# lucidrains/glom-pytorch

Hardware: NVIDIA H100
Metric: column-iterations/sec (BxNxLxiters) at dim=512 L=6 224/14 (higher is better)
Workload: dtype bf16

## Files before the change

glom_pytorch_b200/_native.py:

```python
import ctypes
import os

_PKG = os.path.dirname(os.path.abspath(__file__))
LIB_PATH = os.environ.get("GLOM_B200_LIB") or os.path.join(_PKG, "libglom_b200.so")

ABI_VERSION = 1
PRECISION = {"fp32": 0, "bf16": 1}
PROFILE_KINDS = ("attention", "gemm1_gelu", "gemm2_combine", "prologue", "tokenize")


class Cfg(ctypes.Structure):
    _fields_ = [("struct_size", ctypes.c_uint32), ("dim", ctypes.c_int32), ("levels", ctypes.c_int32),
                ("n", ctypes.c_int32), ("attend_self", ctypes.c_int32), ("mask_side", ctypes.c_int32),
                ("mask_d2_max", ctypes.c_int32), ("precision", ctypes.c_int32)]


class WeightsRef(ctypes.Structure):
    _fields_ = [("struct_size", ctypes.c_uint32)] + [
        (k, ctypes.c_void_p) for k in ("bu_w1", "bu_b1", "bu_w2", "bu_b2", "td_w1", "td_b1", "td_w2", "td_b2")]


class Grads(ctypes.Structure):
    _fields_ = [("struct_size", ctypes.c_uint32)] + [
        (k, ctypes.c_void_p) for k in ("d_tokens", "d_pos", "d_state0", "d_init", "d_bu_w1", "d_bu_b1", "d_bu_w2",
                                       "d_bu_b2", "d_td_w1", "d_td_b1", "d_td_w2", "d_td_b2")]


_vp, _sz, _i32, _f32 = ctypes.c_void_p, ctypes.c_size_t, ctypes.c_int, ctypes.c_float
_CFG, _W, _G = ctypes.POINTER(Cfg), ctypes.POINTER(WeightsRef), ctypes.POINTER(Grads)
_SZP, _I32P = ctypes.POINTER(_sz), ctypes.POINTER(_i32)
_SETTLE = [_CFG, _vp, _vp, _vp, _vp, _vp, _vp, _i32, _i32, _f32, _vp, _vp, _sz, _vp]

SIGNATURES = {
    "glom_b200_abi_version": (_i32, []),
    "glom_b200_last_error": (ctypes.c_char_p, []),
    "glom_b200_packed_weight_bytes": (_i32, [_CFG, _SZP]),
    "glom_b200_pack_weights": (_i32, [_CFG, _W, _vp, _sz, _vp]),
    "glom_b200_workspace_bytes": (_i32, [_CFG, _i32, _i32, _i32, _SZP]),
    "glom_b200_forward": (_i32, [_CFG, _vp, _vp, _vp, _vp, _vp, _vp, _i32, _i32, _i32, _vp, _sz, _vp]),
    "glom_b200_forward_resume": (_i32, [_CFG, _vp, _vp, _vp, _vp, _vp, _i32, _i32, _i32, _vp, _sz, _vp, _i32, _I32P]),
    "glom_b200_settle_workspace_bytes": (_i32, [_CFG, _i32, _i32, _SZP]),
    "glom_b200_settle": (_i32, _SETTLE),
    "glom_b200_settle_all_workspace_bytes": (_i32, [_CFG, _i32, _i32, _SZP]),
    "glom_b200_settle_all": (_i32, _SETTLE),
    "glom_b200_settle_workspace_offset": (_i32, [_CFG, _i32, _i32, _i32, _i32, _SZP, _SZP]),
    "glom_b200_settle_queue_workspace_bytes": (_i32, [_CFG, _i32, _i32, _SZP]),
    "glom_b200_settle_queue_begin": (_i32, [_CFG, _vp, _vp, _vp, _vp, _vp, _vp, _i32, _i32, _i32, _f32, _vp, _sz, _vp]),
    "glom_b200_settle_queue_run": (_i32, [_CFG, _vp, _vp, _vp, _vp, _vp, _vp, _vp, _i32, _i32, _i32, _f32, _vp, _sz, _vp,
                                          _i32, _i32, _vp]),
    "glom_b200_settle_video_workspace_bytes": (_i32, [_CFG, _i32, _i32, _SZP]),
    "glom_b200_settle_video_begin": (_i32, [_CFG, _vp, _vp, _vp, _vp, _vp, _vp, _i32, _i32, _i32, _i32, _f32, _vp, _sz,
                                            _vp]),
    "glom_b200_settle_video_run": (_i32, [_CFG, _vp, _vp, _vp, _vp, _vp, _vp, _vp, _i32, _i32, _i32, _i32, _f32, _vp, _sz,
                                          _vp, _i32, _i32, _vp]),
    "glom_b200_forward_steps_workspace_bytes": (_i32, [_CFG, _i32, _i32, _i32, _SZP]),
    "glom_b200_forward_steps": (_i32, [_CFG, _vp, _vp, _vp, _vp, _vp, _vp, _i32, _vp, _i32, _i32, _vp, _sz, _vp]),
    "glom_b200_tokenize_workspace_bytes": (_i32, [_i32, _i32, _i32, _i32, _i32, _i32, _SZP]),
    "glom_b200_tokenize": (_i32, [_vp, _vp, _vp, _vp, _i32, _i32, _i32, _i32, _i32, _i32, _vp, _sz, _vp]),
    "glom_b200_last_launch_count": (_i32, []),
    "glom_b200_workspace_offset": (_i32, [_CFG, _i32, _i32, _i32, _i32, _SZP, _SZP]),
    "glom_b200_backward_workspace_bytes": (_i32, [_CFG, _i32, _SZP]),
# ... 50 lines not shown
    if rc != 0:
        raise GlomB200Error(f"glom_b200 error {rc}: {load().glom_b200_last_error().decode()}")


def make_cfg(dim, levels, n, attend_self, mask_side, mask_d2_max, precision):
    return Cfg(ctypes.sizeof(Cfg), dim, levels, n, int(bool(attend_self)), mask_side, mask_d2_max,
               PRECISION[precision])


def _bytes(symbol, *args):
    out = ctypes.c_size_t()
    check(getattr(load(), symbol)(*args, ctypes.byref(out)))
    return out.value


def packed_weight_bytes(cfg):
    return _bytes("glom_b200_packed_weight_bytes", ctypes.byref(cfg))


def workspace_bytes(cfg, batch, iters, return_all):
    return _bytes("glom_b200_workspace_bytes", ctypes.byref(cfg), batch, iters, int(return_all))


def workspace_offset(cfg, batch, iters, return_all, which):
    off, nb = ctypes.c_size_t(), ctypes.c_size_t()
    check(load().glom_b200_workspace_offset(ctypes.byref(cfg), batch, iters, int(return_all), which,
                                            ctypes.byref(off), ctypes.byref(nb)))
    return off.value, nb.value


def settle_workspace_offset(cfg, batch, max_iters, return_all, which):
    off, nb = ctypes.c_size_t(), ctypes.c_size_t()
    check(load().glom_b200_settle_workspace_offset(ctypes.byref(cfg), batch, max_iters, int(return_all), which,
                                                   ctypes.byref(off), ctypes.byref(nb)))
    return off.value, nb.value


def pack_weights(cfg, ptrs, packed_ptr, packed_bytes, stream):
    w = WeightsRef(ctypes.sizeof(WeightsRef), *ptrs)
    check(load().glom_b200_pack_weights(ctypes.byref(cfg), ctypes.byref(w), packed_ptr, packed_bytes, stream))


def forward(cfg, packed_ptr, tokens_ptr, pos_ptr, state_in_ptr, init_ptr, out_ptr, batch, iters,
            return_all, ws_ptr, ws_bytes, stream):
    check(load().glom_b200_forward(ctypes.byref(cfg), packed_ptr, tokens_ptr, pos_ptr, state_in_ptr, init_ptr,
                                   out_ptr, batch, iters, int(return_all), ws_ptr, ws_bytes, stream))
# ... 176 lines not shown
```

glom_pytorch_b200/csrc/engine.h:

```cpp
#pragma once
#include <cuda.h>
#include <cuda_runtime.h>
#include <cuda_bf16.h>
#include <stdarg.h>
#include <stddef.h>
#include <stdint.h>
#include <stdio.h>
#include <atomic>
#include <mutex>
#include <vector>

#include "../../include/glom_b200.h"

namespace glom {

enum ProfKind { PROF_ATTN = 0, PROF_GEMM1 = 1, PROF_GEMM2 = 2, PROF_PREP = 3, PROF_TOKENIZE = 4, PROF_KINDS = 5 };
struct Profiler {
  bool enabled = false;
  std::vector<cudaEvent_t> ev;
  size_t used = 0;
  struct Span { int kind; size_t a, b; };
  std::vector<Span> spans;
  size_t mark(cudaStream_t st) {
    if (used == ev.size()) { cudaEvent_t e; cudaEventCreate(&e); ev.push_back(e); }
// ... 22 lines not shown

struct PackedLayout {
  size_t w1_off, w2_off, b1_off, b2_off, total;
};
PackedLayout packed_layout(int d, int L, int precision);

struct WorkspaceLayout {
  size_t s32_off;
  size_t s32_bytes;
  size_t sb_off[2];
  size_t sp_off[2];
  size_t xb_off;
  size_t h_off;
  size_t h_bytes;
  size_t c_off;
  size_t c_bytes;
  size_t nsq_off[2];
  size_t nsq_bytes;
  size_t attn_acc_off;
  size_t attn_acc_bytes;
  size_t total;
};
WorkspaceLayout workspace_layout(const Geometry& g, int precision, int iters, int return_all);

struct SettleLayout {
  WorkspaceLayout fwd;
  size_t dsq_off;
  size_t flags_off;
  size_t frozen_off;
  size_t block_frozen_off;
  size_t done_off;
  size_t level_q_off;
  size_t flags_bytes;
  size_t total;
};
SettleLayout settle_layout(const Geometry& g, int max_iters, int return_all = 0);

struct QueueLayout {
  SettleLayout settle;
  size_t slab_off[2];
  size_t queue_off;
  size_t slot_img_off;
  size_t age_off;
  size_t pending_off;
  size_t gather_off;
  size_t fresh_off;
// ... 6 lines not shown
QueueLayout queue_layout(const Geometry& g, int max_iters);

struct QueueSlots {
  int *slot_img, *age, *pending, *gather_img, *fresh, *block_fresh, *head, *unfinished;
  int images, frames, max_iters;
};

struct Bf16Buffers {
  const float* s32_in;  float* s32_out;
  int s32_in_bcast;
  const __nv_bfloat16* sb_in;  __nv_bfloat16* sb_out;
  const __nv_bfloat16* sp_in;  __nv_bfloat16* sp_out;
  const __nv_bfloat16* xb;
  __nv_bfloat16* h;  __nv_bfloat16* c;
  float* attn_acc;
  const float* nsq_in;  float* nsq_out;
  const float* pos;
  const __nv_bfloat16* w1;  const __nv_bfloat16* w2;  const float* b1;  const float* b2;
  const int* frozen;
  const int* block_frozen;
  float* dsq_out;
  const int* block_fresh;
  int ii_reduce;
};

static inline int rep_h_blocks(int n) {
  int a = n, b = 128;
  while (b) { const int r = a % b; a = b; b = r; }
  return n / a;
}
static inline int rep_row_blocks(int n) { return (rep_h_blocks(n) * 128 + 255) / 256; }

typedef CUresult (*EncodeTiledFn)(CUtensorMap*, CUtensorMapDataType, cuuint32_t, void*, const cuuint64_t*,
                                  const cuuint64_t*, const cuuint32_t*, const cuuint32_t*, CUtensorMapInterleave,
                                  CUtensorMapSwizzle, CUtensorMapL2promotion, CUtensorMapFloatOOBfill);

struct Launch {
  EncodeTiledFn enc; int num_sms; cudaStream_t st; Profiler* prof;
  int launches;
  char err[400];
  int launched(cudaError_t e, const char* what = nullptr) { ++launches; return check(e, what); }
  int launched(const char* what = nullptr) { return launched(cudaGetLastError(), what); }
  int check(cudaError_t e, const char* what = nullptr) {
    if (e == cudaSuccess) return 0;
    return what ? fail(GLOM_B200_ERR_CUDA, "%s: %s", what, cudaGetErrorString(e)) : fail(GLOM_B200_ERR_CUDA, "%s", cudaGetErrorString(e));
  }
// ... 166 lines not shown
```

glom_pytorch_b200/csrc/gemm_sched.cuh:

```cuda
#pragma once
#include "tc_common.cuh"

namespace glom {

struct GemmParams {
  int rows, d, L, n, G;
  int num_m, num_n, num_tiles;
  int m128;
  int z0;
  int n_half;
  const float* bias;
  const float* s32_in;
  int s_bcast;
  const __nv_bfloat16* c_in;
  const float* pos;
  float* s32_out;
  __nv_bfloat16* sb_out;
  __nv_bfloat16* sp_out;
  float* nsq_out;
  int nparts;
  float* tok_out;
  int tok_kb;
  const int* frozen;
  const int* block_frozen;
  float* dsq_out;
  const int* block_fresh;
  int num_m_rep, num_full_tiles;
  unsigned long long full_mask, rep_mask;
  int remap_l, h_period;
};

struct TileInfo {
  int z;
  int m_blk, n_blk;
  int num_kb;
};

__host__ __device__ __forceinline__ int nth_set_bit(unsigned long long m, int k) {
  int z = 0;
  for (;; ++z)
    if ((m >> z) & 1ull) { if (k == 0) return z; --k; }
}

template <int MODE, bool REDUCED = false>
__host__ __device__ __forceinline__ TileInfo decode_tile(const GemmParams& p, int tile) {
  TileInfo t;
  if (REDUCED && p.num_m_rep > 0) {
    const bool full = tile < p.num_full_tiles;
    const int nm = full ? p.num_m : p.num_m_rep;
    const int r = full ? tile / p.num_n : (tile - p.num_full_tiles) / p.num_n;
    t.n_blk = tile % p.num_n;
    t.m_blk = r % nm;
    t.z = nth_set_bit(full ? p.full_mask : p.rep_mask, r / nm);
  } else {
    t.n_blk = tile % p.num_n;
    const int r = tile / p.num_n;
    t.m_blk = r % p.num_m;
    t.z = p.z0 + r / p.num_m;
  }
  if (MODE == 0) t.num_kb = p.d / BK;
  else if (MODE == 1) t.num_kb = ((t.z == p.L - 1) ? 4 * p.d : 8 * p.d) / BK;
  else t.num_kb = p.tok_kb;
  return t;
}

template <int MODE>
__host__ __device__ __forceinline__ int sched_tile(const GemmParams& p, int c, int C, int it) {
  if (MODE != 1) { const int t = c + it * C; return t < p.num_tiles ? t : -1; }
  const int S = p.n_half;
  const int B = p.num_tiles - S;
  const int heavy = B % C;
  const int nb = (B - c + C - 1) / C;
  const int nbig = nb > 0 ? nb : 0;
  if (it < nbig) return c + it * C;
  int k = it - nbig;
  const int light = C - heavy;
  const int first = (2 * light < S) ? 2 * light : S;
  if (c >= heavy) {
    if (k < 2) { const int j = k * light + (c - heavy); if (j < first) return B + j; }
    k -= 2;
    if (k < 0) return -1;
  }
  const int j = first + k * C + c;
  return j < S ? B + j : -1;
}

__host__ __device__ __forceinline__ bool ii_k1_full(int z, int t) { return (z & 1) ? z <= 2 * t - 3 : z <= 2 * t; }
__host__ __device__ __forceinline__ bool ii_k2_full(int l, int t) { return l <= t; }
__host__ __device__ __forceinline__ int ii_k3_full_levels(int t) { return t; }

template <typename Full>
__host__ __forceinline__ void set_reduced(GemmParams& p, int z_end, int num_m_rep, Full full) {
  p.num_m_rep = num_m_rep;
  p.full_mask = p.rep_mask = 0;
  for (int z = p.z0; z < z_end; ++z) (full(z) ? p.full_mask : p.rep_mask) |= 1ull << z;
  p.num_full_tiles = __builtin_popcountll(p.full_mask) * p.num_m * p.num_n;
  p.num_tiles = p.num_full_tiles + __builtin_popcountll(p.rep_mask) * num_m_rep * p.num_n;
}

__host__ __device__ __forceinline__ void attn_item(int it, int full_items, int per_img, int ntiles, int l_full, int& b, int& l) {
  if (it >= full_items) { b = 0; l = l_full + (it - full_items) / ntiles; }
  else { b = it / per_img; l = (it % per_img) / ntiles; }
}

}
```

glom_pytorch_b200/csrc/glom_api.cu:

```cuda
#include "../../include/glom_b200.h"
#include "../../include/glom_b200_tree.h"
#include "engine.h"

#include <mutex>
#include <stdarg.h>
#include <stdio.h>
#include <string.h>

namespace glom {

static thread_local char g_err[512] = "";
static thread_local Profiler g_prof;
static thread_local Launch g_launch{};

static int fail(int code, const char* fmt, ...) {
  va_list ap;
  va_start(ap, fmt);
  vsnprintf(g_err, sizeof(g_err), fmt, ap);
  va_end(ap);
  return code;
}

static bool misaligned(const void* p, size_t a) { return reinterpret_cast<uintptr_t>(p) % a != 0; }

// ... 17 lines not shown
  w.s32_off = off;
  w.s32_bytes = (return_all || iters == 0) ? 0 : state_elems * 4;
  off = align_up(off + w.s32_bytes, 1024);
  if (precision == GLOM_B200_BF16) {
    for (int i = 0; i < 2; ++i) { w.sb_off[i] = off; off = align_up(off + state_elems * 2, 1024); }
    for (int i = 0; i < 2; ++i) { w.sp_off[i] = off; off = align_up(off + (size_t)g.rows * (g.L - 1) * g.d * 2, 1024); }
    w.xb_off = off; off = align_up(off + (size_t)g.rows * g.d * 2, 1024);
    w.h_bytes = (size_t)((g.rows + 127) / 128 * 128) * g.G * 4 * g.d * 2;
    w.c_bytes = state_elems * 2;
    w.nsq_bytes = (size_t)g.rows * g.L * g.nparts * 4;
  } else {
    w.h_bytes = (size_t)g.rows * g.G * 4 * g.d * 4;
    w.c_bytes = state_elems * 4;
    w.nsq_bytes = 0;
  }
  w.h_off = off; off = align_up(off + w.h_bytes, 1024);
  w.c_off = off; off = align_up(off + w.c_bytes, 1024);
  for (int i = 0; i < 2; ++i) { w.nsq_off[i] = off; off = align_up(off + w.nsq_bytes, 1024); }
  w.attn_acc_off = off;
  w.attn_acc_bytes = (precision == GLOM_B200_BF16 && g.n > 576) ? (state_elems + (size_t)g.rows * g.L * 2) * 4 : 0;
  off = align_up(off + w.attn_acc_bytes, 1024);
  w.total = off > 0 ? off : 1024;
  return w;
}

SettleLayout settle_layout(const Geometry& g, int max_iters, int return_all) {
  SettleLayout s{};
  s.fwd = workspace_layout(g, GLOM_B200_BF16, max_iters, return_all);
  size_t off = s.fwd.total;
  s.dsq_off = off; off = align_up(off + s.fwd.nsq_bytes, 1024);
  s.flags_off = off;
  s.frozen_off = off; off = align_up(off + (size_t)g.B * 4, 16);
  s.block_frozen_off = off; off = align_up(off + (size_t)(g.rows + 255) / 256 * 4, 16);
  s.done_off = off; off = align_up(off + 4, 16);
  s.level_q_off = off; off += (size_t)g.B * g.L * 4;
  s.flags_bytes = off - s.flags_off;
  s.total = align_up(off, 1024);
  return s;
}

QueueLayout queue_layout(const Geometry& g, int max_iters) {
  QueueLayout q{};
  q.settle = settle_layout(g, max_iters, 0);
  size_t off = q.settle.total;
  q.slab_off[0] = q.settle.fwd.s32_off;
  q.slab_off[1] = off; off = align_up(off + q.settle.fwd.s32_bytes, 1024);
// ... 108 lines not shown
  return 0;
}

GLOM_B200_API int glom_b200_pack_weights(const glom_b200_cfg* cfg, const glom_b200_weights_ref* w, void* packed, size_t packed_bytes,
                           void* stream) {
  if (int r = check_cfg(cfg)) return r;
  if (!w || w->struct_size != sizeof(glom_b200_weights_ref)) return fail(GLOM_B200_ERR_INVALID, "weights struct missing or wrong size");
  if (!w->bu_w1 || !w->bu_b1 || !w->bu_w2 || !w->bu_b2 || !w->td_w1 || !w->td_b1 || !w->td_w2 || !w->td_b2)
    return fail(GLOM_B200_ERR_INVALID, "a weight pointer is NULL");
  const PackedLayout pl = packed_layout(cfg->dim, cfg->levels, cfg->precision);
  if (!packed || packed_bytes < pl.total) return fail(GLOM_B200_ERR_WORKSPACE, "packed buffer: need %zu bytes, got %zu", pl.total, packed_bytes);
  if (misaligned(packed, 1024)) return fail(GLOM_B200_ERR_INVALID, "packed buffer must be 1024-byte aligned");
  Launch& ln = begin_launch(0, stream);
  if (int r = launch_pack(cfg->dim, cfg->levels, cfg->precision, w->bu_w1, w->bu_b1, w->bu_w2, w->bu_b2, w->td_w1, w->td_b1,
                          w->td_w2, w->td_b2, packed, ln))
    return fail(r, "pack_weights launch: %s", ln.err);
  return 0;
}

GLOM_B200_API int glom_b200_workspace_bytes(const glom_b200_cfg* cfg, int batch, int iters, int return_all, size_t* out_bytes) {
  if (int r = check_cfg(cfg)) return r;
  if (batch < 1 || iters < 0 || !out_bytes) return fail(GLOM_B200_ERR_INVALID, "bad batch/iters/out_bytes");
  *out_bytes = workspace_layout(make_geometry(cfg, batch), cfg->precision, iters, return_all).total;
  return 0;
}

GLOM_B200_API int glom_b200_workspace_offset(const glom_b200_cfg* cfg, int batch, int iters, int return_all, int which,
                               size_t* out_offset, size_t* out_bytes) {
  if (int r = check_cfg(cfg)) return r;
  if (batch < 1 || iters < 0 || !out_offset || !out_bytes) return fail(GLOM_B200_ERR_INVALID, "bad arguments");
  const WorkspaceLayout w = workspace_layout(make_geometry(cfg, batch), cfg->precision, iters, return_all);
  switch (which) {
    case 0: *out_offset = w.h_off; *out_bytes = w.h_bytes; return 0;
    case 1: *out_offset = w.c_off; *out_bytes = w.c_bytes; return 0;
    case 2: *out_offset = w.nsq_off[0]; *out_bytes = w.nsq_bytes; return 0;
    default: return fail(GLOM_B200_ERR_INVALID, "unknown workspace buffer id %d", which);
  }
}


static int check_tensors(const char* pre, bool has_packed, const void* packed_weights, const float* tokens, const float* pos,
                         const float* state_in, const float* init_levels, const float* state_out, const void* workspace) {
  if ((has_packed && !packed_weights) || !tokens || !pos || !state_out)
    return fail(GLOM_B200_ERR_INVALID, "%sa required pointer is NULL", pre);
  if (!state_in && !init_levels) return fail(GLOM_B200_ERR_INVALID, "%sneed state_in or init_levels", pre);
  if (state_in == state_out) return fail(GLOM_B200_ERR_INVALID, "%sstate_out must not alias state_in", pre);
// ... 96 lines not shown
    Bf16Buffers& b = sbuf.step;
    const bool resume = a.resume_parity >= 0;
    const int p0 = resume ? a.resume_parity : 0;
    const bool s0_direct = resume || (!return_all && iters >= 1);
    int prep;
    if (resume) {
      prep = launch_prep(g, nullptr, nullptr, a.pos, a.tokens, nullptr, nullptr, nullptr, sbuf.xb, nullptr, ln);
      if (prep == 0 && return_all)
        prep = ln.launched(cudaMemcpyAsync(state_out, state_in, slab * sizeof(float), cudaMemcpyDeviceToDevice, ln.st));
    } else {
      prep = launch_prep(g, state_in, init_levels, a.pos, a.tokens, s0_direct ? nullptr : loc(0), sbuf.sb[0], sbuf.sp[0], sbuf.xb,
                         sbuf.nsq[0], ln);
    }
    if (prep) return fail(prep, "prep launch: %s", ln.err);
    const SettleFlags fl = freeze ? bind_settle_flags(sl, a.workspace) : SettleFlags{};
    b.frozen = fl.frozen; b.block_frozen = fl.block_frozen;
    b.dsq_out = settle ? fl.dsq : nullptr;
    if (settle) {
      if (int r = ln.check(cudaMemsetAsync(ws + sl.flags_off, 0, sl.flags_bytes, ln.st)))
        return fail(r, "settle flags memset: %s", ln.err);
    }
    const bool ii = !state_in && !resume && !freeze && iters >= g.L + 1 && g.L <= 32 &&
                    rep_row_blocks(g.n) < (g.rows + 255) / 256 && (size_t)g.n * g.L * g.d < (1u << 31);
    for (int t = 0; t < iters; ++t) {
      if (steps) {
        if (int r = launch_steps_schedule(g, t, iters, steps, fl.frozen, fl.block_frozen, ln))
          return fail(r, "step schedule launch before step %d: %s", t, ln.err);
      }
      b.s32_in = (s0_direct && t == 0) ? (state_in ? state_in : init_levels) : loc(t); b.s32_out = loc(t + 1);
      b.s32_in_bcast = (s0_direct && t == 0 && !state_in) ? 1 : 0;
      set_parity(sbuf, (t + p0) & 1);
      b.ii_reduce = ii && t < g.L;
      if (int r = step_bf16(g, b, t, ln)) return fail(r, "step %d: %s", t, ln.err);
      if (settle) {
        if (int r = launch_settle_converge(g, t + 1, settle->tol, fl.dsq, b.nsq_out, fl.frozen, fl.block_frozen, fl.done,
                                           fl.level_q, settle->steps, ln))
          return fail(r, "settle convergence launch after step %d: %s", t, ln.err);
      }
    }
    const int32_t* image_steps = settle ? settle->steps : steps;
    if (ii && return_all) {
      if (int r = launch_level_fill(g, state_out, ln)) return fail(r, "return_all level fill launch: %s", ln.err);
    }
    if (image_steps && return_all) {
      if (int r = launch_steps_fill(g, iters, image_steps, state_out, ln)) return fail(r, "return_all fill launch: %s", ln.err);
    } else if (image_steps && iters > 0) {
// ... 596 lines not shown
```

glom_pytorch_b200/csrc/ptx.cuh:

```cuda
#pragma once
#include <cuda.h>
#include <cuda_runtime.h>
#include <cuda_bf16.h>
#include <stdint.h>
#include <stdio.h>

namespace glom {

#ifndef GLOM_WAIT_TIMEOUT_CYCLES
#define GLOM_WAIT_TIMEOUT_CYCLES (4000000000LL)
#endif

__device__ __forceinline__ uint32_t smem_u32(const void* p) {
  return static_cast<uint32_t>(__cvta_generic_to_shared(p));
}

__device__ __forceinline__ void mbar_init(uint64_t* bar, uint32_t count) {
  asm volatile("mbarrier.init.shared::cta.b64 [%0], %1;" ::"r"(smem_u32(bar)), "r"(count) : "memory");
}
__device__ __forceinline__ void fence_barrier_init() {
  asm volatile("fence.mbarrier_init.release.cluster;" ::: "memory");
}
__device__ __forceinline__ void mbar_arrive_expect_tx(uint64_t* bar, uint32_t bytes) {
  asm volatile("mbarrier.arrive.expect_tx.shared::cta.b64 _, [%0], %1;" ::"r"(smem_u32(bar)), "r"(bytes)
// ... 60 lines not shown

__device__ __forceinline__ void red_add_f32x4(float* dst, float4 v) {
  asm volatile("red.global.add.v4.f32 [%0], {%1, %2, %3, %4};" ::"l"(dst), "f"(v.x), "f"(v.y), "f"(v.z), "f"(v.w)
               : "memory");
}

__device__ __forceinline__ uint64_t wgmma_desc_sw128(uint32_t saddr, uint32_t lbo_bytes, uint32_t sbo_bytes) {
  uint64_t d = 0;
  d |= static_cast<uint64_t>((saddr & 0x3FFFFu) >> 4);
  d |= static_cast<uint64_t>((lbo_bytes >> 4) & 0x3FFFu) << 16;
  d |= static_cast<uint64_t>((sbo_bytes >> 4) & 0x3FFFu) << 32;
  d |= static_cast<uint64_t>(1) << 62;
  return d;
}
__device__ __forceinline__ void wgmma_fence() { asm volatile("wgmma.fence.sync.aligned;" ::: "memory"); }
__device__ __forceinline__ void wgmma_commit() { asm volatile("wgmma.commit_group.sync.aligned;" ::: "memory"); }
template <int N>
__device__ __forceinline__ void wgmma_wait() { asm volatile("wgmma.wait_group.sync.aligned %0;" ::"n"(N) : "memory"); }
template <int R>
__device__ __forceinline__ void wgmma_fence_regs(float (&d)[R]) {
#pragma unroll
  for (int i = 0; i < R; ++i) asm volatile("" : "+f"(d[i])::"memory");
}

template <int TA, int TB>
__device__ __forceinline__ void wgmma_n64(float (&d)[32], uint64_t adesc, uint64_t bdesc) {
  asm volatile(
      "{\n\t"
      "wgmma.mma_async.sync.aligned.m64n64k16.f32.bf16.bf16 "
      "{%0, %1, %2, %3, %4, %5, %6, %7, %8, %9, %10, %11, %12, %13, %14, %15, %16, %17, %18, %19, %20, %21, %22, %23, %24, %25, %26, %27, %28, %29, %30, %31}, "
      "%32, %33, 1, 1, 1, %34, %35;\n\t}"
      : "+f"(d[0]), "+f"(d[1]), "+f"(d[2]), "+f"(d[3]), "+f"(d[4]), "+f"(d[5]), "+f"(d[6]), "+f"(d[7]), "+f"(d[8]), "+f"(d[9]), "+f"(d[10]), "+f"(d[11]), "+f"(d[12]), "+f"(d[13]), "+f"(d[14]), "+f"(d[15]), "+f"(d[16]), "+f"(d[17]), "+f"(d[18]), "+f"(d[19]), "+f"(d[20]), "+f"(d[21]), "+f"(d[22]), "+f"(d[23]), "+f"(d[24]), "+f"(d[25]), "+f"(d[26]), "+f"(d[27]), "+f"(d[28]), "+f"(d[29]), "+f"(d[30]), "+f"(d[31])
      : "l"(adesc), "l"(bdesc), "n"(TA), "n"(TB));
}
template <int TA, int TB>
__device__ __forceinline__ void wgmma_n128(float (&d)[64], uint64_t adesc, uint64_t bdesc) {
  asm volatile(
      "{\n\t"
      "wgmma.mma_async.sync.aligned.m64n128k16.f32.bf16.bf16 "
      "{%0, %1, %2, %3, %4, %5, %6, %7, %8, %9, %10, %11, %12, %13, %14, %15, %16, %17, %18, %19, %20, %21, %22, %23, %24, %25, %26, %27, %28, %29, %30, %31, %32, %33, %34, %35, %36, %37, %38, %39, %40, %41, %42, %43, %44, %45, %46, %47, %48, %49, %50, %51, %52, %53, %54, %55, %56, %57, %58, %59, %60, %61, %62, %63}, "
      "%64, %65, 1, 1, 1, %66, %67;\n\t}"
      : "+f"(d[0]), "+f"(d[1]), "+f"(d[2]), "+f"(d[3]), "+f"(d[4]), "+f"(d[5]), "+f"(d[6]), "+f"(d[7]), "+f"(d[8]), "+f"(d[9]), "+f"(d[10]), "+f"(d[11]), "+f"(d[12]), "+f"(d[13]), "+f"(d[14]), "+f"(d[15]), "+f"(d[16]), "+f"(d[17]), "+f"(d[18]), "+f"(d[19]), "+f"(d[20]), "+f"(d[21]), "+f"(d[22]), "+f"(d[23]), "+f"(d[24]), "+f"(d[25]), "+f"(d[26]), "+f"(d[27]), "+f"(d[28]), "+f"(d[29]), "+f"(d[30]), "+f"(d[31]), "+f"(d[32]), "+f"(d[33]), "+f"(d[34]), "+f"(d[35]), "+f"(d[36]), "+f"(d[37]), "+f"(d[38]), "+f"(d[39]), "+f"(d[40]), "+f"(d[41]), "+f"(d[42]), "+f"(d[43]), "+f"(d[44]), "+f"(d[45]), "+f"(d[46]), "+f"(d[47]), "+f"(d[48]), "+f"(d[49]), "+f"(d[50]), "+f"(d[51]), "+f"(d[52]), "+f"(d[53]), "+f"(d[54]), "+f"(d[55]), "+f"(d[56]), "+f"(d[57]), "+f"(d[58]), "+f"(d[59]), "+f"(d[60]), "+f"(d[61]), "+f"(d[62]), "+f"(d[63])
      : "l"(adesc), "l"(bdesc), "n"(TA), "n"(TB));
}
template <int TA, int TB>
__device__ __forceinline__ void wgmma_n256(float (&d)[128], uint64_t adesc, uint64_t bdesc) {
// ... 132 lines not shown
```

glom_pytorch_b200/csrc/tc_kernels.cu:

```cuda
#include "gemm_sched.cuh"
#include "tc_common.cuh"

#include <stdio.h>
#include <stdlib.h>
#include <string.h>

#include <type_traits>

namespace glom {

constexpr int GEMM_CONSUMER_WARPS = 8;
constexpr int GEMM_THREADS = 128 + 32 * GEMM_CONSUMER_WARPS;
constexpr uint32_t GEMM_PRODUCER_REGS = 40;
constexpr uint32_t GEMM_CONSUMER_REGS = 232;

__device__ unsigned long long g_kernel_clk[PROF_KINDS][8];


template <int MODE, int BN>
struct GemmCfg {
  static constexpr int PARTS = (BN == 256) ? 4 : 2;
  static constexpr int PART_COLS = BN / PARTS;
  static constexpr int THREADS = GEMM_THREADS;
  static constexpr uint32_t B_STAGE_BYTES = BN * BK * 2;
// ... 91 lines not shown
        const TileInfo t = decode_tile<MODE, RED>(p, tile);
        if constexpr (SETTLE) { if (settle_skip<MODE>(p, t)) continue; }
        const CUtensorMap* amap;
        int a_col, b_row;
        if (MODE == 0) {
          const int l = t.z >> 1;
          if (t.z == 0) { amap = &map_a0; a_col = 0; }
          else if (t.z & 1) { amap = &map_a2; a_col = l * p.d; }
          else { amap = &map_a1; a_col = (l - 1) * p.d; }
          b_row = t.z * 4 * p.d + t.n_blk * BN;
        } else if (MODE == 1) {
          amap = &map_a0; a_col = 0;
          b_row = t.z * p.d + t.n_blk * BN;
        } else {
          amap = &map_a0; a_col = 0;
          b_row = t.n_blk * BN;
        }
        const int a_row = t.m_blk * 256 + cta_rank * BM;
        const int blk0 = (2 * t.z * p.m128 + (a_row >> 7)) * kbg_n;
        int td_skip = blk_skip;
        if constexpr (RED && MODE == 1) {
          if (p.num_m_rep > 0 && t.z + 1 >= p.remap_l) td_skip -= ((a_row >> 7) - (a_row >> 7) % p.h_period) * kbg_n;
        }
        for (int kb = 0; kb < t.num_kb; ++kb) {
          GLOM_CNT_WAIT(w0, mbar_wait(&empty_bar[stage], phase ^ 1));
          if (elected) {
            const uint32_t sa = smem0 + (uint32_t)stage * Cfg::STAGE_BYTES;
            uint64_t* bar = &full_bar[stage];
            mbar_arrive_expect_tx(bar, Cfg::STAGE_BYTES);
            if (MODE == 1) {
              const int blk = blk0 + kb + (kb >= kbg_n ? td_skip : 0);
              tma_load_2d_hint(sa, amap, bar, 0, blk * BM, pol_first);
            } else {
              tma_load_2d(sa, amap, bar, a_col + kb * BK, a_row);
            }
            const uint32_t b_half = (uint32_t)cta_rank * (BN / 2);
            tma_load_2d_multicast(sa + A_STAGE_BYTES + b_half * BK * 2, &map_b, bar, kb * BK, b_row + (int)b_half, 0x3);
          }
          __syncwarp();
          if (++stage == STAGES) { stage = 0; phase ^= 1; }
        }
      }
      if (cnt_cta && elected) atomicAdd(&cnt[4], w0);
    }
  } else {
    setmaxnreg_inc<GEMM_CONSUMER_REGS>();
    const int cw = warp - W_CONSUMER0;
// ... 14 lines not shown
      if (lane == 0) { mbar_arrive(&empty_bar[slot]); mbar_arrive_cluster(empty_peer + 8u * (uint32_t)slot); }
    };
    int stage = 0; uint32_t phase = 0;
    float acc[BN / 2];
    for (int it = 0, tile; (tile = sched_tile<MODE>(p, cluster_id, num_clusters, it)) >= 0; ++it) {
      const TileInfo t = decode_tile<MODE, RED>(p, tile);
      if constexpr (SETTLE) { if (settle_skip<MODE>(p, t)) continue; }
      const int row0 = t.m_blk * 256 + cta_rank * BM + pair * 32;
      const int rows_left = p.rows - row0;
      uint32_t live = ~0u;
      if constexpr (SETTLE && MODE == 1)
        live = __ballot_sync(0xffffffffu, row0 + lane < p.rows && !p.frozen[(row0 + lane) / p.n]);
      bool remap = false;
      if constexpr (RED && MODE == 1) remap = p.num_m_rep > 0 && t.z >= p.remap_l;
      if (MODE == 1 && lane < rows_left) {
        const int src_row = remap ? (row0 + lane) % p.n : row0 + lane;
        const size_t o = ((size_t)src_row * p.L + t.z) * p.d + t.n_blk * BN + x * (BN / 2);
#pragma unroll
        for (int c = 0; c < BN / 2; c += 32) {
          if (!p.s_bcast) prefetch_l2(p.s32_in + o + c);
          if ((c & 63) == 0) prefetch_l2(p.c_in + o + c);
        }
      }
#pragma unroll
      for (int i = 0; i < BN / 2; ++i) acc[i] = 0.f;
      int prev = -1;
      for (int kb = 0; kb < t.num_kb; ++kb) {
        GLOM_CNT_WAIT(w0, mbar_wait(&full_bar[stage], phase));
        const uint32_t sa = smem0 + (uint32_t)stage * Cfg::STAGE_BYTES;
        wgmma_fence_regs(acc);
        wgmma_fence();
        wgmma_kblock<BN, 0>(acc, sa + (uint32_t)wg * (A_STAGE_BYTES / 2), sa + A_STAGE_BYTES);
        wgmma_commit();
        wgmma_wait<1>();
        wgmma_fence_regs(acc);
        if (prev >= 0) release(prev);
        prev = stage;
        if (++stage == STAGES) { stage = 0; phase ^= 1; }
      }
      wgmma_wait<0>();
      wgmma_fence_regs(acc);
      release(prev);
      const long long busy_t0 = cnt_cta ? clock64() : 0;
      if constexpr (MODE == 0) {
        const int wrow0 = t.m_blk * 256 + cta_rank * BM + 64 * wg;
        if (wrow0 < p.rows) {
          const int hblk0 = (t.z * p.m128 + (t.m_blk * 2 + cta_rank)) * (4 * p.d / BK) + t.n_blk * (BN / BK);
          const float* bias = p.bias + (size_t)t.z * 4 * p.d + t.n_blk * BN + 2 * (lane & 3);
          uint32_t pk[BN / 4];
#pragma unroll
          for (int s = 0; s < BN / 64; ++s) {
#pragma unroll
            for (int j = 0; j < 8; ++j) {
              const float2 b = __ldg(reinterpret_cast<const float2*>(bias + 64 * s + 8 * j));
#pragma unroll
              for (int h = 0; h < 2; ++h)
                pk[16 * s + 2 * j + h] = gelu_pair_bf16(acc[4 * (8 * s + j) + 2 * h], acc[4 * (8 * s + j) + 2 * h + 1], b.x, b.y);
// ... 710 lines not shown
  GLOM_TRY(map2d(ln, &mh, b.h, h_rows, BK, BM, "H"));
  GLOM_TRY(map2d(ln, &mh_out, b.h, h_rows, BK, 64, "H out"));
  CUtensorMap mx, msb, msp, mw1, mw2;
  GLOM_TRY(map2d(ln, &mx, b.xb, rows, d, BM, "Xb"));
  GLOM_TRY(map2d(ln, &msb, b.sb_in, rows, (uint64_t)L * d, BM, "Sb"));
  GLOM_TRY(map2d(ln, &msp, b.sp_in, rows, (uint64_t)(L - 1) * d, BM, "Sp"));
  GLOM_TRY(map2d(ln, &mw1, b.w1, (uint64_t)g.G * 4 * d, d, 128, "W1p"));
  GLOM_TRY(map2d(ln, &mw2, b.w2, (uint64_t)L * d, (uint64_t)8 * d, (uint32_t)g.bn2 / 2, "W2p"));
  {
    GemmParams p{};
    p.rows = rows; p.d = d; p.L = L; p.n = n; p.G = g.G;
    p.z0 = (step_index > 0 && g.G > 1 && !b.block_fresh) ? 1 : 0;
    p.num_m = (rows + 255) / 256; p.num_n = 4 * d / 256; p.num_tiles = (g.G - p.z0) * p.num_m * p.num_n;
    p.bias = b.b1; p.m128 = m128;
    p.frozen = b.frozen; p.block_frozen = b.block_frozen; p.block_fresh = b.block_fresh;
    if (b.ii_reduce) set_reduced(p, g.G, rep_row_blocks(n), [&](int z) { return ii_k1_full(z, step_index); });
    ProfScope scope(ln.prof, PROF_GEMM1, st);
    GLOM_TRY(ln.launched(launch_gemm<0, 256>(mx, msb, msp, mw1, mh_out, p, num_sms, st), "gemm1 launch"));
  }
  GLOM_TRY(launch_attention(g, b, b.ii_reduce ? ii_k3_full_levels(step_index) : L, ln));
  {
    GemmParams p{};
    p.rows = rows; p.d = d; p.L = L; p.n = n; p.G = g.G;
    p.num_m = (rows + 255) / 256; p.num_n = d / g.bn2; p.z0 = 0; p.num_tiles = L * p.num_m * p.num_n;
    p.n_half = p.num_m * p.num_n;
    p.m128 = m128;
    p.bias = b.b2; p.s32_in = b.s32_in; p.s_bcast = b.s32_in_bcast; p.c_in = b.c; p.pos = b.pos;
    p.s32_out = b.s32_out; p.sb_out = b.sb_out; p.sp_out = b.sp_out; p.nsq_out = b.nsq_out; p.nparts = g.nparts;
    p.frozen = b.frozen; p.block_frozen = b.block_frozen; p.dsq_out = b.dsq_out;
    if (b.ii_reduce) {
      set_reduced(p, L, rep_row_blocks(n), [&](int l) { return ii_k2_full(l, step_index); });
      p.n_half = (L - 1 <= step_index ? p.num_m : p.num_m_rep) * p.num_n;
      p.remap_l = step_index; p.h_period = rep_h_blocks(n);
    }
    cudaError_t e;
    ProfScope scope(ln.prof, PROF_GEMM2, st);
    if (g.bn2 == 256) e = launch_gemm<1, 256>(mh, mh, mh, mw2, mh, p, num_sms, st);
    else if (g.bn2 == 128) e = launch_gemm<1, 128>(mh, mh, mh, mw2, mh, p, num_sms, st);
    else e = launch_gemm<1, 64>(mh, mh, mh, mw2, mh, p, num_sms, st);
    GLOM_TRY(ln.launched(e, "gemm2 launch"));
  }
  return 0;
}


int tokenize_tc(const __nv_bfloat16* patches, const __nv_bfloat16* wtok, const float* bias, float* tokens, int rows,
                int d, int kp, Launch& ln) {
  const int num_sms = ln.num_sms;
  cudaStream_t st = ln.st;
  const int bn = (d % 256 == 0) ? 256 : (d % 128 == 0) ? 128 : 64;
  CUtensorMap ma, mb;
  GLOM_TRY(map2d(ln, &ma, patches, rows, kp, BM, "patches"));
  GLOM_TRY(map2d(ln, &mb, wtok, d, kp, (uint32_t)bn / 2, "Wtok"));
  GemmParams p{};
  p.rows = rows; p.d = d; p.L = 1; p.n = 1; p.G = 1;
  p.num_m = (rows + 255) / 256; p.num_n = d / bn; p.num_tiles = p.num_m * p.num_n;
  p.bias = bias; p.tok_out = tokens; p.tok_kb = kp / BK;
// ... 9 lines not shown
```

glom_pytorch_b200/glom.py:

```python
from math import prod, sqrt

import operator
import weakref

import torch
from torch import nn

from . import _native


def _aligned_bytes(nbytes, device, align=1024):
    raw = torch.empty(nbytes + align, dtype=torch.uint8, device=device)
    off = (-raw.data_ptr()) % align
    return raw[off:off + nbytes]


def _contiguous16(t):
    t = t.contiguous()
    return t if t.data_ptr() % 16 == 0 else t.clone()


def _capturing():
    return (not torch.compiler.is_compiling() and torch.cuda.is_available()
            and torch.cuda.is_current_stream_capturing())
# ... 448 lines not shown
        else:
            resume, self._resume = self._resume, None
        plain = steps is None and tol is None
        with torch.cuda.device(device):
            stream = torch.cuda.current_stream(device).cuda_stream
            pos_key = (self.pos_emb.weight.data_ptr(), self.pos_emb.weight._version)
            call_key = (device.index, stream, b, n, self.precision, pos_key)
            use_resume = (plain and allow_resume and resume is not None and state_in is not None and iters >= 1
                          and self.precision == "bf16" and resume["ref"]() is state_in
                          and state_in._version == resume["version"] and resume["key"] == call_key)
            tokens = _contiguous16(tokens.detach().to(torch.float32))
            pos = _contiguous16(pos.detach().to(torch.float32))
            init = _contiguous16(init.detach().to(torch.float32))
            if state_in is not None:
                state_in = _contiguous16(state_in.detach().to(device=device, dtype=torch.float32))
            state_ptr = None if state_in is None else state_in.data_ptr()
            cfg = self.engine_cfg(n)
            packed = self._packed_weights(cfg, device, stream)
            shape = (b, n, self.levels, self.dim)
            out = torch.empty(((iters + 1,) + shape) if return_all else shape, dtype=torch.float32, device=device)
            if tol is not None:
                steps = torch.empty(b, dtype=torch.int32, device=device)
            if plain:
                ws_bytes = _native.workspace_bytes(cfg, b, iters, return_all)
            elif tol is None:
                ws_bytes = _native.forward_steps_workspace_bytes(cfg, b, iters, return_all)
            else:
                ws_bytes = (_native.settle_all_workspace_bytes if return_all else _native.settle_workspace_bytes)(cfg, b, iters)
            ws = self._get_workspace(ws_bytes, device)
            if tol is not None:
                _native.settle(cfg, packed.data_ptr(), tokens.data_ptr(), pos.data_ptr(), state_ptr, init.data_ptr(),
                               out.data_ptr(), b, iters, return_all, tol, steps.data_ptr(), ws.data_ptr(), ws.numel(), stream)
            elif steps is not None:
                _native.forward_steps(cfg, packed.data_ptr(), tokens.data_ptr(), pos.data_ptr(), state_ptr, init.data_ptr(),
                                      out.data_ptr(), b, steps.data_ptr(), iters, return_all, ws.data_ptr(), ws.numel(),
                                      stream)
            elif use_resume and ws.data_ptr() == resume["ws"]:
                parity = _native.forward_resume(cfg, packed.data_ptr(), tokens.data_ptr(), pos.data_ptr(), state_ptr,
                                                out.data_ptr(), b, iters, return_all, ws.data_ptr(), ws.numel(), stream,
                                                resume["parity"])
            else:
                parity = iters & 1
                _native.forward(cfg, packed.data_ptr(), tokens.data_ptr(), pos.data_ptr(), state_ptr, init.data_ptr(),
                                out.data_ptr(), b, iters, return_all, ws.data_ptr(), ws.numel(), stream)
            self.last_launches = _native.last_launch_count() + getattr(self, "_tok_launches", 0)
            if plain and allow_resume and not return_all and iters >= 1 and self.precision == "bf16":
                self._resume = {"ref": weakref.ref(out), "version": out._version, "key": call_key, "ws": ws.data_ptr(),
# ... 216 lines not shown
```

glom_pytorch_b200/ops.py:

```python
import weakref

import torch
from torch import Tensor

from . import _native
from .glom import _aligned_bytes, _contiguous16, radius_mask_d2

_GRADS = ("d_tokens", "d_pos", "d_state0", "d_init", "d_bu_w1", "d_bu_b1", "d_bu_w2", "d_bu_b2", "d_td_w1", "d_td_b1",
          "d_td_w2", "d_td_b2")


def _stream(device):
    return torch.cuda.current_stream(device).cuda_stream


def _f32(t):
    return _contiguous16(t.detach().to(torch.float32))


_checked_masks = {}


def _check_mask(mask, side, d2_max):
    _require(mask.dim() == 3 and tuple(mask.shape) == (1, side * side, side * side) and mask.dtype == torch.bool,
# ... 83 lines not shown
    with torch.cuda.device(device):
        stream = _stream(device)
        tokens, pos, init = _f32(tokens), _f32(pos), _f32(init_levels)
        state0 = None if state0 is None else _f32(state0)
        state_ptr = None if state0 is None else state0.data_ptr()
        cfg = _native.make_cfg(dim, levels, n, attend_self, mask_side, mask_d2_max, precision)
        packed = _packed(cfg, weights, device)
        shape = (b, n, levels, dim)
        out = torch.empty(((iters + 1,) + shape) if engine_all else shape, dtype=torch.float32, device=device)
        if tol is not None:
            steps = torch.empty(b, dtype=torch.int32, device=device)
            nbytes = (_native.settle_all_workspace_bytes if engine_all else _native.settle_workspace_bytes)(cfg, b, iters)
            ws = _aligned_bytes(nbytes, device)
            _native.settle(cfg, packed.data_ptr(), tokens.data_ptr(), pos.data_ptr(), state_ptr, init.data_ptr(),
                           out.data_ptr(), b, iters, engine_all, tol, steps.data_ptr(), ws.data_ptr(), ws.numel(), stream)
            return out, steps
        if steps is not None:
            steps = steps.to(device=device, dtype=torch.int32).contiguous()
            ws = _aligned_bytes(_native.forward_steps_workspace_bytes(cfg, b, iters, engine_all), device)
            _native.forward_steps(cfg, packed.data_ptr(), tokens.data_ptr(), pos.data_ptr(), state_ptr, init.data_ptr(),
                                  out.data_ptr(), b, steps.data_ptr(), iters, engine_all, ws.data_ptr(), ws.numel(),
                                  stream)
        else:
            ws = _aligned_bytes(_native.workspace_bytes(cfg, b, iters, engine_all), device)
            _native.forward(cfg, packed.data_ptr(), tokens.data_ptr(), pos.data_ptr(), state_ptr, init.data_ptr(),
                            out.data_ptr(), b, iters, engine_all, ws.data_ptr(), ws.numel(), stream)
    return out


@torch.library.custom_op("glom_b200::check_radius_mask", mutates_args=(), tags=(torch.Tag.cudagraph_unsafe,))
def check_radius_mask(mask: Tensor, mask_side: int, mask_d2_max: int) -> Tensor:
    _check_mask(mask, mask_side, mask_d2_max)
    return torch.empty(0, dtype=torch.bool, device=mask.device)


@check_radius_mask.register_fake
def _(mask, mask_side, mask_d2_max):
    return mask.new_empty((0,), dtype=torch.bool)


@torch.library.custom_op("glom_b200::tokenize", mutates_args=())
def tokenize(img: Tensor, weight: Tensor, bias: Tensor, patch: int, precision: str) -> Tensor:
    _check_image_args(img, weight, patch)
    _check_floats(img.device, img=img, weight=weight, bias=bias)
    _check_shape("bias", bias, weight.shape[:1])
    img = img.detach().float().contiguous()
    b, _, h, w = img.shape
# ... 236 lines not shown
```

include/glom_b200.h:

```cpp
#ifndef GLOM_B200_H_
#define GLOM_B200_H_

#include <stddef.h>
#include <stdint.h>

#ifdef __cplusplus
extern "C" {
#endif

#define GLOM_B200_ABI_VERSION 1

#if defined(__GNUC__)
#define GLOM_B200_API __attribute__((visibility("default")))
#else
#define GLOM_B200_API
#endif

typedef enum glom_b200_status {
  GLOM_B200_OK = 0,
  GLOM_B200_ERR_INVALID = -1,
  GLOM_B200_ERR_WORKSPACE = -2,
  GLOM_B200_ERR_CUDA = -3,
  GLOM_B200_ERR_DEVICE = -4
} glom_b200_status;
// ... 11 lines not shown
  int32_t attend_self;
  int32_t mask_side;
  int32_t mask_d2_max;
  int32_t precision;
} glom_b200_cfg;

typedef struct glom_b200_weights_ref {
  uint32_t struct_size;
  const float* bu_w1; const float* bu_b1; const float* bu_w2; const float* bu_b2;
  const float* td_w1; const float* td_b1; const float* td_w2; const float* td_b2;
} glom_b200_weights_ref;

GLOM_B200_API int glom_b200_abi_version(void);

GLOM_B200_API const char* glom_b200_last_error(void);

GLOM_B200_API int glom_b200_packed_weight_bytes(const glom_b200_cfg* cfg, size_t* out_bytes);

GLOM_B200_API int glom_b200_pack_weights(const glom_b200_cfg* cfg, const glom_b200_weights_ref* w,
                           void* packed, size_t packed_bytes, void* stream);

GLOM_B200_API int glom_b200_workspace_bytes(const glom_b200_cfg* cfg, int batch, int iters,
                              int return_all, size_t* out_bytes);

GLOM_B200_API int glom_b200_forward(const glom_b200_cfg* cfg, const void* packed_weights,
                      const float* tokens, const float* pos, const float* state_in,
                      const float* init_levels, float* state_out, int batch, int iters,
                      int return_all, void* workspace, size_t workspace_bytes, void* stream);

GLOM_B200_API int glom_b200_forward_resume(const glom_b200_cfg* cfg, const void* packed_weights, const float* tokens,
                                           const float* pos, const float* state_in, float* state_out, int batch, int iters,
                                           int return_all, void* workspace, size_t workspace_bytes, void* stream,
                                           int shadow_parity, int* out_shadow_parity);

GLOM_B200_API int glom_b200_settle_workspace_bytes(const glom_b200_cfg* cfg, int batch, int max_iters, size_t* out_bytes);
GLOM_B200_API int glom_b200_settle(const glom_b200_cfg* cfg, const void* packed_weights, const float* tokens, const float* pos,
                                   const float* state_in, const float* init_levels, float* state_out, int batch,
                                   int max_iters, float tol, int32_t* steps_out, void* workspace, size_t workspace_bytes,
                                   void* stream);
GLOM_B200_API int glom_b200_settle_all_workspace_bytes(const glom_b200_cfg* cfg, int batch, int max_iters, size_t* out_bytes);
GLOM_B200_API int glom_b200_settle_all(const glom_b200_cfg* cfg, const void* packed_weights, const float* tokens,
                                       const float* pos, const float* state_in, const float* init_levels, float* states_out,
                                       int batch, int max_iters, float tol, int32_t* steps_out, void* workspace,
                                       size_t workspace_bytes, void* stream);

GLOM_B200_API int glom_b200_forward_steps_workspace_bytes(const glom_b200_cfg* cfg, int batch, int max_steps, int return_all,
// ... 100 lines not shown
```

Measured before the change: 67.90 million.

## Cache level-0 bottom-up GEMM2 partial sums across iterations

Level 0's bottom-up contribution depends only on the fixed token input. On the first step the GEMM2 mainloop writes its fp32 accumulator after the first 4d of K to a new workspace slab. On later steps, level-0 tiles preload that partial and run only the remaining K blocks. A new workspace-size entry point reserves the slab, and the tile scheduler, the K-start offset and the host code are reworked to support it. The cost is extra fp32 reads and writes of the partial, plus a full wgmma drain at the store point on step 0.

```diff
diff --git a/glom_pytorch_b200/_native.py b/glom_pytorch_b200/_native.py
--- a/glom_pytorch_b200/_native.py
+++ b/glom_pytorch_b200/_native.py
@@ -37,6 +37,7 @@
     "glom_b200_packed_weight_bytes": (_i32, [_CFG, _SZP]),
     "glom_b200_pack_weights": (_i32, [_CFG, _W, _vp, _sz, _vp]),
     "glom_b200_workspace_bytes": (_i32, [_CFG, _i32, _i32, _i32, _SZP]),
+    "glom_b200_workspace_bytes_with_partial": (_i32, [_CFG, _i32, _i32, _i32, _SZP]),
     "glom_b200_forward": (_i32, [_CFG, _vp, _vp, _vp, _vp, _vp, _vp, _i32, _i32, _i32, _vp, _sz, _vp]),
     "glom_b200_forward_resume": (_i32, [_CFG, _vp, _vp, _vp, _vp, _vp, _i32, _i32, _i32, _vp, _sz, _vp, _i32, _I32P]),
     "glom_b200_settle_workspace_bytes": (_i32, [_CFG, _i32, _i32, _SZP]),
@@ -133,6 +134,10 @@
     return _bytes("glom_b200_workspace_bytes", ctypes.byref(cfg), batch, iters, int(return_all))
 
 
+def workspace_bytes_with_partial(cfg, batch, iters, return_all):
+    return _bytes("glom_b200_workspace_bytes_with_partial", ctypes.byref(cfg), batch, iters, int(return_all))
+
+
 def workspace_offset(cfg, batch, iters, return_all, which):
     off, nb = ctypes.c_size_t(), ctypes.c_size_t()
     check(load().glom_b200_workspace_offset(ctypes.byref(cfg), batch, iters, int(return_all), which,
diff --git a/glom_pytorch_b200/csrc/engine.h b/glom_pytorch_b200/csrc/engine.h
--- a/glom_pytorch_b200/csrc/engine.h
+++ b/glom_pytorch_b200/csrc/engine.h
@@ -68,6 +68,7 @@
   size_t total;
 };
 WorkspaceLayout workspace_layout(const Geometry& g, int precision, int iters, int return_all);
+size_t bu0_partial_bytes(const Geometry& g, int precision, int iters);
 
 struct SettleLayout {
   WorkspaceLayout fwd;
@@ -120,6 +121,7 @@
   float* dsq_out;
   const int* block_fresh;
   int ii_reduce;
+  float* bu0_partial;
 };
 
 static inline int rep_h_blocks(int n) {
diff --git a/glom_pytorch_b200/csrc/gemm_sched.cuh b/glom_pytorch_b200/csrc/gemm_sched.cuh
--- a/glom_pytorch_b200/csrc/gemm_sched.cuh
+++ b/glom_pytorch_b200/csrc/gemm_sched.cuh
@@ -28,12 +28,15 @@
   int num_m_rep, num_full_tiles;
   unsigned long long full_mask, rep_mask;
   int remap_l, h_period;
+  float* bu0_partial;
+  int bu0_mode;
 };
 
 struct TileInfo {
   int z;
   int m_blk, n_blk;
   int num_kb;
+  int kb0;
 };
 
 __host__ __device__ __forceinline__ int nth_set_bit(unsigned long long m, int k) {
@@ -45,7 +48,11 @@
 template <int MODE, bool REDUCED = false>
 __host__ __device__ __forceinline__ TileInfo decode_tile(const GemmParams& p, int tile) {
   TileInfo t;
-  if (REDUCED && p.num_m_rep > 0) {
+  const int n0 = (MODE == 1 && REDUCED && p.bu0_mode == 2) ? p.num_m * p.num_n : 0;
+  if (n0 > 0 && tile >= p.num_tiles - n0) {
+    const int r = tile - (p.num_tiles - n0);
+    t.z = 0; t.m_blk = r / p.num_n; t.n_blk = r % p.num_n;
+  } else if (REDUCED && p.num_m_rep > 0) {
     const bool full = tile < p.num_full_tiles;
     const int nm = full ? p.num_m : p.num_m_rep;
     const int r = full ? tile / p.num_n : (tile - p.num_full_tiles) / p.num_n;
@@ -58,9 +65,11 @@
     t.m_blk = r % p.num_m;
     t.z = p.z0 + r / p.num_m;
   }
+  t.kb0 = 0;
   if (MODE == 0) t.num_kb = p.d / BK;
   else if (MODE == 1) t.num_kb = ((t.z == p.L - 1) ? 4 * p.d : 8 * p.d) / BK;
   else t.num_kb = p.tok_kb;
+  if (n0 > 0 && t.z == 0) { t.kb0 = 4 * p.d / BK; t.num_kb = 4 * p.d / BK; }
   return t;
 }
 
@@ -98,6 +107,20 @@
   p.num_tiles = p.num_full_tiles + __builtin_popcountll(p.rep_mask) * num_m_rep * p.num_n;
 }
 
+__host__ __forceinline__ void set_k2_tiles(GemmParams& p, int t, bool reduced, int bu0_mode) {
+  const int level_tiles = p.num_m * p.num_n;
+  p.bu0_mode = bu0_mode;
+  p.z0 = bu0_mode == 2 ? 1 : 0;
+  p.num_tiles = (p.L - p.z0) * level_tiles;
+  p.n_half = level_tiles;
+  if (reduced) {
+    set_reduced(p, p.L, rep_row_blocks(p.n), [&](int l) { return ii_k2_full(l, t); });
+    p.n_half = (p.L - 1 <= t ? p.num_m : p.num_m_rep) * p.num_n;
+    p.remap_l = t; p.h_period = rep_h_blocks(p.n);
+  }
+  if (bu0_mode == 2) { p.num_tiles += level_tiles; p.n_half += level_tiles; }
+}
+
 __host__ __device__ __forceinline__ void attn_item(int it, int full_items, int per_img, int ntiles, int l_full, int& b, int& l) {
   if (it >= full_items) { b = 0; l = l_full + (it - full_items) / ntiles; }
   else { b = it / per_img; l = (it % per_img) / ntiles; }
diff --git a/glom_pytorch_b200/csrc/glom_api.cu b/glom_pytorch_b200/csrc/glom_api.cu
--- a/glom_pytorch_b200/csrc/glom_api.cu
+++ b/glom_pytorch_b200/csrc/glom_api.cu
@@ -63,6 +63,11 @@
   off = align_up(off + w.attn_acc_bytes, 1024);
   w.total = off > 0 ? off : 1024;
   return w;
+}
+
+size_t bu0_partial_bytes(const Geometry& g, int precision, int iters) {
+  if (precision != GLOM_B200_BF16 || iters < 2) return 0;
+  return align_up((size_t)(g.rows + 255) / 256 * 256 * g.d * 4, 1024);
 }
 
 SettleLayout settle_layout(const Geometry& g, int max_iters, int return_all) {
@@ -217,6 +222,15 @@
   if (int r = check_cfg(cfg)) return r;
   if (batch < 1 || iters < 0 || !out_bytes) return fail(GLOM_B200_ERR_INVALID, "bad batch/iters/out_bytes");
   *out_bytes = workspace_layout(make_geometry(cfg, batch), cfg->precision, iters, return_all).total;
+  return 0;
+}
+
+GLOM_B200_API int glom_b200_workspace_bytes_with_partial(const glom_b200_cfg* cfg, int batch, int iters, int return_all,
+                                                         size_t* out_bytes) {
+  if (int r = check_cfg(cfg)) return r;
+  if (batch < 1 || iters < 0 || !out_bytes) return fail(GLOM_B200_ERR_INVALID, "bad batch/iters/out_bytes");
+  const Geometry g = make_geometry(cfg, batch);
+  *out_bytes = workspace_layout(g, cfg->precision, iters, return_all).total + bu0_partial_bytes(g, cfg->precision, iters);
   return 0;
 }
 
@@ -359,6 +373,8 @@
     }
     const bool ii = !state_in && !resume && !freeze && iters >= g.L + 1 && g.L <= 32 &&
                     rep_row_blocks(g.n) < (g.rows + 255) / 256 && (size_t)g.n * g.L * g.d < (1u << 31);
+    const size_t bu0_bytes = freeze ? 0 : bu0_partial_bytes(g, cfg->precision, iters);
+    if (bu0_bytes && a.workspace_bytes >= wl.total + bu0_bytes) b.bu0_partial = reinterpret_cast<float*>(ws + wl.total);
     for (int t = 0; t < iters; ++t) {
       if (steps) {
         if (int r = launch_steps_schedule(g, t, iters, steps, fl.frozen, fl.block_frozen, ln))
diff --git a/glom_pytorch_b200/csrc/ptx.cuh b/glom_pytorch_b200/csrc/ptx.cuh
--- a/glom_pytorch_b200/csrc/ptx.cuh
+++ b/glom_pytorch_b200/csrc/ptx.cuh
@@ -106,6 +106,16 @@
 #pragma unroll
   for (int i = 0; i < R; ++i) asm volatile("" : "+f"(d[i])::"memory");
 }
+__device__ __forceinline__ void acc_init4(float& a, float& b, float& c, float& d, const void* src, bool load) {
+  asm volatile(
+      "{\n\t.reg .pred q;\n\t"
+      "setp.ne.b32 q, %5, 0;\n\t"
+      "mov.b32 %0, 0;\n\tmov.b32 %1, 0;\n\tmov.b32 %2, 0;\n\tmov.b32 %3, 0;\n\t"
+      "@q ld.global.cs.v4.f32 {%0, %1, %2, %3}, [%4];\n\t}"
+      : "=f"(a), "=f"(b), "=f"(c), "=f"(d)
+      : "l"(src), "r"((int)load)
+      : "memory");
+}
 
 template <int TA, int TB>
 __device__ __forceinline__ void wgmma_n64(float (&d)[32], uint64_t adesc, uint64_t bdesc) {
diff --git a/glom_pytorch_b200/csrc/tc_kernels.cu b/glom_pytorch_b200/csrc/tc_kernels.cu
--- a/glom_pytorch_b200/csrc/tc_kernels.cu
+++ b/glom_pytorch_b200/csrc/tc_kernels.cu
@@ -137,7 +137,7 @@
         if constexpr (RED && MODE == 1) {
           if (p.num_m_rep > 0 && t.z + 1 >= p.remap_l) td_skip -= ((a_row >> 7) - (a_row >> 7) % p.h_period) * kbg_n;
         }
-        for (int kb = 0; kb < t.num_kb; ++kb) {
+        for (int kb = t.kb0; kb < t.kb0 + t.num_kb; ++kb) {
           GLOM_CNT_WAIT(w0, mbar_wait(&empty_bar[stage], phase ^ 1));
           if (elected) {
             const uint32_t sa = smem0 + (uint32_t)stage * Cfg::STAGE_BYTES;
@@ -198,8 +198,24 @@
           if ((c & 63) == 0) prefetch_l2(p.c_in + o + c);
         }
       }
-#pragma unroll
-      for (int i = 0; i < BN / 2; ++i) acc[i] = 0.f;
+      float4* bu0 = nullptr;
+      int bu0_store_kb = -1;
+      if constexpr (RED && MODE == 1) {
+        if (p.bu0_mode != 0 && t.z == 0) {
+          bu0 = reinterpret_cast<float4*>(p.bu0_partial) +
+                ((size_t)(t.m_blk * p.num_n + t.n_blk) * 2 + cta_rank) * (BN / 8) * 256 + (threadIdx.x - 128);
+          if (p.bu0_mode == 1) bu0_store_kb = 4 * p.d / BK - 1;
+        }
+      }
+      if constexpr (RED && MODE == 1) {
+        const bool load = t.kb0 > 0;
+#pragma unroll
+        for (int j = 0; j < BN / 8; ++j)
+          acc_init4(acc[4 * j], acc[4 * j + 1], acc[4 * j + 2], acc[4 * j + 3], bu0 + (size_t)j * 256, load);
+      } else {
+#pragma unroll
+        for (int i = 0; i < BN / 2; ++i) acc[i] = 0.f;
+      }
       int prev = -1;
       for (int kb = 0; kb < t.num_kb; ++kb) {
         GLOM_CNT_WAIT(w0, mbar_wait(&full_bar[stage], phase));
@@ -208,7 +224,15 @@
         wgmma_fence();
         wgmma_kblock<BN, 0>(acc, sa + (uint32_t)wg * (A_STAGE_BYTES / 2), sa + A_STAGE_BYTES);
         wgmma_commit();
-        wgmma_wait<1>();
+        if (RED && MODE == 1 && kb == bu0_store_kb) {
+          wgmma_wait<0>();
+          wgmma_fence_regs(acc);
+#pragma unroll
+          for (int j = 0; j < BN / 8; ++j)
+            __stcg(bu0 + (size_t)j * 256, make_float4(acc[4 * j], acc[4 * j + 1], acc[4 * j + 2], acc[4 * j + 3]));
+        } else {
+          wgmma_wait<1>();
+        }
         wgmma_fence_regs(acc);
         if (prev >= 0) release(prev);
         prev = stage;
@@ -965,17 +989,14 @@
   {
     GemmParams p{};
     p.rows = rows; p.d = d; p.L = L; p.n = n; p.G = g.G;
-    p.num_m = (rows + 255) / 256; p.num_n = d / g.bn2; p.z0 = 0; p.num_tiles = L * p.num_m * p.num_n;
-    p.n_half = p.num_m * p.num_n;
+    p.num_m = (rows + 255) / 256; p.num_n = d / g.bn2;
+    const int bu0_mode = (b.bu0_partial && !b.block_frozen && !b.block_fresh) ? (step_index == 0 ? 1 : 2) : 0;
+    set_k2_tiles(p, step_index, b.ii_reduce != 0, bu0_mode);
+    p.bu0_partial = b.bu0_partial;
     p.m128 = m128;
     p.bias = b.b2; p.s32_in = b.s32_in; p.s_bcast = b.s32_in_bcast; p.c_in = b.c; p.pos = b.pos;
     p.s32_out = b.s32_out; p.sb_out = b.sb_out; p.sp_out = b.sp_out; p.nsq_out = b.nsq_out; p.nparts = g.nparts;
     p.frozen = b.frozen; p.block_frozen = b.block_frozen; p.dsq_out = b.dsq_out;
-    if (b.ii_reduce) {
-      set_reduced(p, L, rep_row_blocks(n), [&](int l) { return ii_k2_full(l, step_index); });
-      p.n_half = (L - 1 <= step_index ? p.num_m : p.num_m_rep) * p.num_n;
-      p.remap_l = step_index; p.h_period = rep_h_blocks(n);
-    }
     cudaError_t e;
     ProfScope scope(ln.prof, PROF_GEMM2, st);
     if (g.bn2 == 256) e = launch_gemm<1, 256>(mh, mh, mh, mw2, mh, p, num_sms, st);
diff --git a/glom_pytorch_b200/glom.py b/glom_pytorch_b200/glom.py
--- a/glom_pytorch_b200/glom.py
+++ b/glom_pytorch_b200/glom.py
@@ -494,7 +494,7 @@
             if tol is not None:
                 steps = torch.empty(b, dtype=torch.int32, device=device)
             if plain:
-                ws_bytes = _native.workspace_bytes(cfg, b, iters, return_all)
+                ws_bytes = _native.workspace_bytes_with_partial(cfg, b, iters, return_all)
             elif tol is None:
                 ws_bytes = _native.forward_steps_workspace_bytes(cfg, b, iters, return_all)
             else:
diff --git a/glom_pytorch_b200/ops.py b/glom_pytorch_b200/ops.py
--- a/glom_pytorch_b200/ops.py
+++ b/glom_pytorch_b200/ops.py
@@ -129,7 +129,7 @@
                                   out.data_ptr(), b, steps.data_ptr(), iters, engine_all, ws.data_ptr(), ws.numel(),
                                   stream)
         else:
-            ws = _aligned_bytes(_native.workspace_bytes(cfg, b, iters, engine_all), device)
+            ws = _aligned_bytes(_native.workspace_bytes_with_partial(cfg, b, iters, engine_all), device)
             _native.forward(cfg, packed.data_ptr(), tokens.data_ptr(), pos.data_ptr(), state_ptr, init.data_ptr(),
                             out.data_ptr(), b, iters, engine_all, ws.data_ptr(), ws.numel(), stream)
     return out
diff --git a/include/glom_b200.h b/include/glom_b200.h
--- a/include/glom_b200.h
+++ b/include/glom_b200.h
@@ -57,6 +57,9 @@
 
 GLOM_B200_API int glom_b200_workspace_bytes(const glom_b200_cfg* cfg, int batch, int iters,
                               int return_all, size_t* out_bytes);
+
+GLOM_B200_API int glom_b200_workspace_bytes_with_partial(const glom_b200_cfg* cfg, int batch, int iters,
+                                                         int return_all, size_t* out_bytes);
 
 GLOM_B200_API int glom_b200_forward(const glom_b200_cfg* cfg, const void* packed_weights,
                       const float* tokens, const float* pos, const float* state_in,
```

Result: faster. 69.41 million, median of 6 (+2.2%).
